# NUS-HPC-AI-Lab/VideoSys

Measured on AMD Instinct MI355X. Metric: videos/min (Open-Sora 512x512x64f, 30 denoise steps, DiT denoising only) + sec/denoise-step, higher is better.
Workload: dtype bf16; 1 GPU; open-sora-v1.2 STDiT3-XL/2 512x512x64f, latent [4,19,64,64], CFG batch 2 = 38912 token rows, 300 text tokens, depth 28; steps_per_video=30, parallelism=dsp1

## Files before the change

### videosys_amd/csrc/rowwise.hip

```cpp
#include "common.h"

#include <cstdlib>
#include "vsys_internal.h"

namespace vsys {
namespace {

template <int MAXV>
__global__ __launch_bounds__(256) void adaln_modulate_kernel(const bf16_t* __restrict__ x, const bf16_t* __restrict__ shift,
                                                             const bf16_t* __restrict__ scale, bf16_t* __restrict__ y,
                                                             int64_t rows, int C, int64_t rows_per_sample,
                                                             int64_t mod_stride, float eps) {
  const int lane = threadIdx.x & 63;
  const int64_t row = (int64_t)blockIdx.x * 4 + (threadIdx.x >> 6);
  if (row >= rows) return;
  const int nchunk = C >> 3;
  const bf16_t* xr = x + row * C;
  float v[MAXV][8];
  float s = 0.f;
#pragma unroll
  for (int i = 0; i < MAXV; ++i) {
    const int c = lane + 64 * i;
    if (c < nchunk) {
      uint4 u = *reinterpret_cast<const uint4*>(xr + c * 8);
      unpack8(u, v[i]);
#pragma unroll
      for (int e = 0; e < 8; ++e) s += v[i][e];
    }
  }
  const float mean = wave_sum(s) / (float)C;
  float q = 0.f;
#pragma unroll
  for (int i = 0; i < MAXV; ++i) {
    const int c = lane + 64 * i;
    if (c < nchunk) {
#pragma unroll
      for (int e = 0; e < 8; ++e) {
        float d = v[i][e] - mean;
        q += d * d;
      }
    }
  }
  const float rstd = rsqrtf(wave_sum(q) / (float)C + eps);
  const int64_t b = row / rows_per_sample;
  const bf16_t* sh = shift + b * mod_stride;
  const bf16_t* sc = scale + b * mod_stride;
  bf16_t* yr = y + row * C;
#pragma unroll
  for (int i = 0; i < MAXV; ++i) {
    const int c = lane + 64 * i;
    if (c < nchunk) {
      float a[8], m[8], o[8];
      unpack8(*reinterpret_cast<const uint4*>(sh + c * 8), a);
      unpack8(*reinterpret_cast<const uint4*>(sc + c * 8), m);
#pragma unroll
      for (int e = 0; e < 8; ++e) o[e] = (v[i][e] - mean) * rstd * (1.0f + m[e]) + a[e];
      *reinterpret_cast<uint4*>(yr + c * 8) = pack8(o);
    }
  }
}

template <int RPW>
__global__ __launch_bounds__(256) void adaln_modulate_rows_kernel(const bf16_t* __restrict__ x, const bf16_t* __restrict__ shift,
                                                                  const bf16_t* __restrict__ scale, bf16_t* __restrict__ y,
                                                                  int64_t rows, int C, int64_t rows_per_sample,
                                                                  int64_t mod_stride, float eps) {
  constexpr int MAXV = 3;
  const int lane = threadIdx.x & 63;
  const int64_t row0 = ((int64_t)blockIdx.x * 4 + (threadIdx.x >> 6)) * RPW;
  if (row0 >= rows) return;
  const int nchunk = C >> 3;
  uint4 u[RPW][MAXV];
#pragma unroll
  for (int r = 0; r < RPW; ++r) {
    const int64_t row = row0 + r < rows ? row0 + r : rows - 1;
#pragma unroll
    for (int i = 0; i < MAXV; ++i) {
      const int c = lane + 64 * i;
      u[r][i] = c < nchunk ? *reinterpret_cast<const uint4*>(x + row * C + c * 8) : make_uint4(0, 0, 0, 0);
    }
  }
  const int64_t b = row0 / rows_per_sample;
  uint4 ush[MAXV], usc[MAXV];
#pragma unroll
  for (int i = 0; i < MAXV; ++i) {
    const int c = lane + 64 * i;
    ush[i] = c < nchunk ? *reinterpret_cast<const uint4*>(shift + b * mod_stride + c * 8) : make_uint4(0, 0, 0, 0);
    usc[i] = c < nchunk ? *reinterpret_cast<const uint4*>(scale + b * mod_stride + c * 8) : make_uint4(0, 0, 0, 0);
  }
#pragma unroll
  for (int r = 0; r < RPW; ++r) {
    float v[MAXV][8];
    float s = 0.f;
#pragma unroll
    for (int i = 0; i < MAXV; ++i) {
      unpack8(u[r][i], v[i]);
      if (lane + 64 * i < nchunk) {
#pragma unroll
        for (int e = 0; e < 8; ++e) s += v[i][e];
      }
    }
    const float mean = wave_sum(s) / (float)C;
    float q = 0.f;
#pragma unroll
    for (int i = 0; i < MAXV; ++i) {
      if (lane + 64 * i < nchunk) {
#pragma unroll
        for (int e = 0; e < 8; ++e) {
          float d = v[i][e] - mean;
          q += d * d;
        }
      }
    }
    const float rstd = rsqrtf(wave_sum(q) / (float)C + eps);
    if (row0 + r < rows) {
#pragma unroll
      for (int i = 0; i < MAXV; ++i) {
        const int c = lane + 64 * i;
        if (c < nchunk) {
          float a[8], m[8], o[8];
          unpack8(ush[i], a);
          unpack8(usc[i], m);
#pragma unroll
          for (int e = 0; e < 8; ++e) o[e] = (v[i][e] - mean) * rstd * (1.0f + m[e]) + a[e];
          *reinterpret_cast<uint4*>(y + (row0 + r) * C + c * 8) = pack8(o);
        }
      }
    }
  }
}

template <int MAXV>
__global__ __launch_bounds__(256) void ln_modulate_kernel(const bf16_t* __restrict__ x, const bf16_t* __restrict__ ln_w,
                                                          const bf16_t* __restrict__ ln_b, const bf16_t* __restrict__ shift,
                                                          const bf16_t* __restrict__ scale, bf16_t* __restrict__ y, int64_t rows,
                                                          int C, int64_t rows_per_sample, int64_t mod_stride, int64_t seg_split,
                                                          int64_t mod_alt, float eps) {
  const int lane = threadIdx.x & 63;
  const int64_t row = (int64_t)blockIdx.x * 4 + (threadIdx.x >> 6);
  if (row >= rows) return;
  const int nchunk = C >> 3;
  const bf16_t* xr = x + row * C;
  float v[MAXV][8];
  float s = 0.f;
#pragma unroll
  for (int i = 0; i < MAXV; ++i) {
    const int c = lane + 64 * i;
    if (c < nchunk) {
      unpack8(*reinterpret_cast<const uint4*>(xr + c * 8), v[i]);
#pragma unroll
      for (int e = 0; e < 8; ++e) s += v[i][e];
    }
  }
  const float mean = wave_sum(s) / (float)C;
  float q = 0.f;
#pragma unroll
  for (int i = 0; i < MAXV; ++i) {
    const int c = lane + 64 * i;
    if (c < nchunk) {
#pragma unroll
      for (int e = 0; e < 8; ++e) {
        const float d = v[i][e] - mean;
        q += d * d;
      }
    }
  }
  const float rstd = rsqrtf(wave_sum(q) / (float)C + eps);
  const int64_t b = row / rows_per_sample;
  const int64_t alt = (seg_split > 0 && row - b * rows_per_sample < seg_split) ? mod_alt : 0;
  bf16_t* yr = y + row * C;
#pragma unroll
  for (int i = 0; i < MAXV; ++i) {
    const int c = lane + 64 * i;
    if (c < nchunk) {
      float o[8];
#pragma unroll
      for (int e = 0; e < 8; ++e) o[e] = (v[i][e] - mean) * rstd;
      if (ln_w != nullptr) {
        float w[8], bb[8];
        unpack8(*reinterpret_cast<const uint4*>(ln_w + c * 8), w);
        unpack8(*reinterpret_cast<const uint4*>(ln_b + c * 8), bb);
#pragma unroll
        for (int e = 0; e < 8; ++e) o[e] = o[e] * w[e] + bb[e];
      }
      if (shift != nullptr) {
        float a[8], m[8];
        unpack8(*reinterpret_cast<const uint4*>(shift + b * mod_stride + alt + c * 8), a);
        unpack8(*reinterpret_cast<const uint4*>(scale + b * mod_stride + alt + c * 8), m);
#pragma unroll
        for (int e = 0; e < 8; ++e) o[e] = o[e] * (1.0f + m[e]) + a[e];
      }
      *reinterpret_cast<uint4*>(yr + c * 8) = pack8(o);
    }
  }
}

__global__ void gate_add_rows_kernel(bf16_t* __restrict__ x, const bf16_t* __restrict__ y, const bf16_t* __restrict__ gate,
                                     int64_t rows, int C8, int64_t rows_per_sample, int64_t gate_stride, int64_t seg_split,
                                     int64_t gate_alt) {
  const int64_t total = rows * C8;
  for (int64_t i = (int64_t)blockIdx.x * blockDim.x + threadIdx.x; i < total; i += (int64_t)gridDim.x * blockDim.x) {
    const int64_t r = i / C8;
    const int c = (int)(i - r * C8);
    const int64_t b = r / rows_per_sample;
    const int64_t alt = (seg_split > 0 && r - b * rows_per_sample < seg_split) ? gate_alt : 0;
    float a[8], v[8], g[8];
    unpack8(reinterpret_cast<const uint4*>(x)[i], a);
    unpack8(reinterpret_cast<const uint4*>(y)[i], v);
    unpack8(*reinterpret_cast<const uint4*>(gate + b * gate_stride + alt + c * 8), g);
#pragma unroll
    for (int k = 0; k < 8; ++k) a[k] += bf2f(f2bf(g[k] * v[k]));
    reinterpret_cast<uint4*>(x)[i] = pack8(a);
  }
}

__global__ void im2col_patch_kernel(const float* __restrict__ z, int Bz, bf16_t* __restrict__ out, int B, int F, int Cin, int H,
                                    int W, int p) {
  const int Hp = H / p, Wp = W / p, K = Cin * p * p;
  const int64_t total = (int64_t)B * F * Hp * Wp * K;
  for (int64_t i = (int64_t)blockIdx.x * blockDim.x + threadIdx.x; i < total; i += (int64_t)gridDim.x * blockDim.x) {
    const int k = (int)(i % K);
    const int64_t tok = i / K;
    const int wp = (int)(tok % Wp), hp = (int)((tok / Wp) % Hp), f = (int)((tok / ((int64_t)Wp * Hp)) % F);
    const int b = (int)(tok / ((int64_t)Wp * Hp * F));
    const int dx = k % p, dy = (k / p) % p, c = k / (p * p);
    out[i] = f2bf(z[((((int64_t)(b % Bz) * F + f) * Cin + c) * H + hp * p + dy) * W + wp * p + dx]);
  }
}

__global__ void unpatchify_cvx_kernel(const bf16_t* __restrict__ x, int64_t ldx, float* __restrict__ out, int B, int F, int Hp,
                                      int Wp, int Cout, int p) {
  const int H = Hp * p, W = Wp * p;
  const int64_t total = (int64_t)B * F * Cout * H * W;
  for (int64_t i = (int64_t)blockIdx.x * blockDim.x + threadIdx.x; i < total; i += (int64_t)gridDim.x * blockDim.x) {
    const int w = (int)(i % W), h = (int)((i / W) % H), c = (int)((i / ((int64_t)W * H)) % Cout);
    const int64_t bf = i / ((int64_t)W * H * Cout);
    const int64_t tok = (bf * Hp + h / p) * Wp + w / p;
    out[i] = bf2f(x[tok * ldx + (c * p + h % p) * p + w % p]);
  }
}

__global__ void mod_table_kernel(const bf16_t* __restrict__ table, const bf16_t* __restrict__ t_mlp, bf16_t* __restrict__ out,
                                 int nblk, int B, int C6) {
  const int64_t i = (int64_t)blockIdx.x * blockDim.x + threadIdx.x;
  const int64_t total = (int64_t)nblk * B * C6;
  if (i >= total) return;
  const int c = (int)(i % C6);
  const int b = (int)((i / C6) % B);
  const int k = (int)(i / ((int64_t)C6 * B));
  out[i] = f2bf(bf2f(table[(int64_t)k * C6 + c]) + bf2f(t_mlp[(int64_t)b * C6 + c]));
}

__global__ void timestep_embedding_kernel(const float* __restrict__ t, bf16_t* __restrict__ out, int B, int dim) {
  const int i = blockIdx.x * blockDim.x + threadIdx.x;
  const int half = dim / 2;
  if (i >= B * half) return;
  const int b = i / half, k = i - b * half;
  const float f = expf(-9.210340371976184f * (float)k / (float)half);
  const float a = t[b] * f;
  out[(int64_t)b * dim + k] = f2bf(cosf(a));
  out[(int64_t)b * dim + half + k] = f2bf(sinf(a));
}

__global__ __launch_bounds__(256) void patch_embed_kernel(const float* __restrict__ x, int Bz, const bf16_t* __restrict__ w,
                                                          const bf16_t* __restrict__ bias, const bf16_t* __restrict__ pos,
                                                          bf16_t* __restrict__ out, int B, int Cin, int T, int H, int W,
                                                          int ph, int pw, int C, int s0, int Sl) {
  const int Hp = (H + ph - 1) / ph, Wp = (W + pw - 1) / pw;
  const int S = Hp * Wp;
  const int cchunks = C >> 3;
  const int64_t total = (int64_t)B * T * Sl * cchunks;
  const int64_t i = (int64_t)blockIdx.x * blockDim.x + threadIdx.x;
  if (i >= total) return;
  const int cc = (int)(i % cchunks);
  const int64_t tok = i / cchunks;
  const int s = s0 + (int)(tok % Sl);
  const int t = (int)((tok / Sl) % T);
  const int b = (int)(tok / ((int64_t)Sl * T));
  const int bz = b % Bz;
  if (s >= S) {
    *reinterpret_cast<uint4*>(out + tok * C + cc * 8) = make_uint4(0, 0, 0, 0);
    return;
  }
  const int hp = s / Wp, wp = s - hp * Wp;
  float acc[8];
  {
    float bb[8];
    unpack8(*reinterpret_cast<const uint4*>(bias + cc * 8), bb);
#pragma unroll
    for (int e = 0; e < 8; ++e) acc[e] = bb[e];
  }
  const int K = Cin * ph * pw;
  if (K == 16) {
    float xin[16];
#pragma unroll
    for (int k = 0; k < 16; ++k) {
      const int ci = k >> 2, dy = (k >> 1) & 1, dx = k & 1;
      const int hh = hp * 2 + dy, ww = wp * 2 + dx;
      xin[k] = 0.f;
      if (ph == 2 && pw == 2 && hh < H && ww < W) xin[k] = bf2f(f2bf(x[((((int64_t)bz * Cin + ci) * T + t) * H + hh) * W + ww]));
    }
    if (ph == 2 && pw == 2) {
#pragma unroll
      for (int e = 0; e < 8; ++e) {
        const bf16_t* wr = w + (int64_t)(cc * 8 + e) * 16;
        float wa[8], wb[8];
        unpack8(*reinterpret_cast<const uint4*>(wr), wa);
        unpack8(*reinterpret_cast<const uint4*>(wr + 8), wb);
#pragma unroll
        for (int k = 0; k < 8; ++k) acc[e] += xin[k] * wa[k] + xin[k + 8] * wb[k];
      }
    }
  }
  if (!(K == 16 && ph == 2 && pw == 2)) {
    for (int ci = 0; ci < Cin; ++ci)
      for (int dy = 0; dy < ph; ++dy)
        for (int dx = 0; dx < pw; ++dx) {
          const int hh = hp * ph + dy, ww = wp * pw + dx;
          float xv = 0.f;
          if (hh < H && ww < W) xv = bf2f(f2bf(x[((((int64_t)bz * Cin + ci) * T + t) * H + hh) * W + ww]));
          const int k = (ci * ph + dy) * pw + dx;
#pragma unroll
          for (int e = 0; e < 8; ++e) acc[e] += xv * bf2f(w[(int64_t)(cc * 8 + e) * K + k]);
        }
  }
  float pp[8];
  unpack8(*reinterpret_cast<const uint4*>(pos + (int64_t)s * C + cc * 8), pp);
#pragma unroll
  for (int e = 0; e < 8; ++e) acc[e] = bf2f(f2bf(acc[e])) + pp[e];
  *reinterpret_cast<uint4*>(out + tok * C + cc * 8) = pack8(acc);
}

template <int MAXV>
__global__ __launch_bounds__(256) void final_layer_kernel(const bf16_t* __restrict__ x, const bf16_t* __restrict__ table,
                                                          const bf16_t* __restrict__ tvec, const bf16_t* __restrict__ w,
                                                          const bf16_t* __restrict__ bias, float* __restrict__ out,
                                                          int B, int T, int Hp, int Wp, int H, int W, int ph, int pw,
                                                          int Cout, int C, float eps, int Sl, float* __restrict__ tokens) {
  const int lane = threadIdx.x & 63;
  const int S = Sl;
  const int64_t rows = (int64_t)B * T * S;
  const int64_t row = (int64_t)blockIdx.x * 4 + (threadIdx.x >> 6);
  if (row >= rows) return;
  const int nchunk = C >> 3;
  const bf16_t* xr = x + row * C;
  float v[MAXV][8];
  float s = 0.f;
#pragma unroll
  for (int i = 0; i < MAXV; ++i) {
    const int c = lane + 64 * i;
    if (c < nchunk) {
      unpack8(*reinterpret_cast<const uint4*>(xr + c * 8), v[i]);
#pragma unroll
      for (int e = 0; e < 8; ++e) s += v[i][e];
    } else {
#pragma unroll
      for (int e = 0; e < 8; ++e) v[i][e] = 0.f;
    }
  }
  const float mean = wave_sum(s) / (float)C;
  float q = 0.f;
#pragma unroll
  for (int i = 0; i < MAXV; ++i) {
    const int c = lane + 64 * i;
    if (c < nchunk) {
#pragma unroll
      for (int e = 0; e < 8; ++e) {
        float d = v[i][e] - mean;
        q += d * d;
      }
    }
  }
  const float rstd = rsqrtf(wave_sum(q) / (float)C + eps);
  const int b = (int)(row / ((int64_t)T * S));
#pragma unroll
  for (int i = 0; i < MAXV; ++i) {
    const int c = lane + 64 * i;
    if (c < nchunk) {
      float sh[8], sc[8], tt[8];
      unpack8(*reinterpret_cast<const uint4*>(table + c * 8), sh);
      unpack8(*reinterpret_cast<const uint4*>(table + C + c * 8), sc);
      unpack8(*reinterpret_cast<const uint4*>(tvec + (int64_t)b * C + c * 8), tt);
#pragma unroll
      for (int e = 0; e < 8; ++e) {
        const float shift = bf2f(f2bf(sh[e] + tt[e])), scale = bf2f(f2bf(sc[e] + tt[e]));
        v[i][e] = bf2f(f2bf((v[i][e] - mean) * rstd * (1.0f + scale) + shift));
      }
    }
  }
  const int NOUT = ph * pw * Cout;
  const int64_t tok = row % ((int64_t)T * S);
  const int t = (int)(tok / S), sidx = (int)(tok % S);
  const int hp = sidx / Wp, wp = sidx - hp * Wp;
  for (int n = 0; n < NOUT; ++n) {
    const bf16_t* wr = w + (int64_t)n * C;
    float d = 0.f;
#pragma unroll
    for (int i = 0; i < MAXV; ++i) {
      const int c = lane + 64 * i;
      if (c < nchunk) {
        float ww[8];
        unpack8(*reinterpret_cast<const uint4*>(wr + c * 8), ww);
#pragma unroll
        for (int e = 0; e < 8; ++e) d += v[i][e] * ww[e];
      }
    }
    d = wave_sum(d);
    if (lane == 0) {
      d = bf2f(f2bf(d + bf2f(bias[n])));
      if (tokens != nullptr) {
        tokens[row * NOUT + n] = d;
        continue;
      }
      const int co = n % Cout;
      const int dx = (n / Cout) % pw, dy = n / (Cout * pw);
      const int hh = hp * ph + dy, ww2 = wp * pw + dx;
      if (hh < H && ww2 < W) out[((((int64_t)b * Cout + co) * T + t) * H + hh) * W + ww2] = d;
    }
  }
}

__global__ void unpatchify_tokens_kernel(const float* __restrict__ tok, float* __restrict__ out, int P, int B, int T, int Sl,
                                         int Hp, int Wp, int H, int W, int ph, int pw, int Cout) {
  const int NOUT = ph * pw * Cout;
  const int64_t total = (int64_t)B * Cout * T * H * W;
  const int64_t i = (int64_t)blockIdx.x * blockDim.x + threadIdx.x;
  if (i >= total) return;
  const int ww = (int)(i % W), hh = (int)((i / W) % H), t = (int)((i / ((int64_t)W * H)) % T);
  const int co = (int)((i / ((int64_t)W * H * T)) % Cout), b = (int)(i / ((int64_t)W * H * T * Cout));
  const int hp = hh / ph, dy = hh - hp * ph, wp = ww / pw, dx = ww - wp * pw;
  const int s = hp * Wp + wp;
  const int r = s / Sl, j = s - r * Sl;
  const int n = (dy * pw + dx) * Cout + co;
  out[i] = tok[((((int64_t)r * B + b) * T + t) * Sl + j) * NOUT + n];
}

__global__ void cfg_euler_kernel(float* __restrict__ z, const float* __restrict__ model_out, int Bz, int Cin, int Cout,
                                 int64_t thw, float guidance, float dt) {
  const int64_t i = (int64_t)blockIdx.x * blockDim.x + threadIdx.x;
  const int64_t total = (int64_t)Bz * Cin * thw;
  if (i >= total) return;
  const int64_t sp = i % thw;
  const int c = (int)((i / thw) % Cin);
  const int b = (int)(i / (thw * Cin));
  const float cond = model_out[((int64_t)b * Cout + c) * thw + sp];
  const float unc = model_out[((int64_t)(b + Bz) * Cout + c) * thw + sp];
  z[i] = z[i] + (unc + guidance * (cond - unc)) * dt;
}

__global__ void cfg_axpby_kernel(float* __restrict__ z, const float* __restrict__ model_out, int Bz, int Cin, int Cout,
                                 int64_t thw, float guidance, float c_z, float c_eps, int cond_first) {
  const int64_t i = (int64_t)blockIdx.x * blockDim.x + threadIdx.x;
  const int64_t total = (int64_t)Bz * Cin * thw;
  if (i >= total) return;
  const int64_t sp = i % thw;
  const int c = (int)((i / thw) % Cin);
  const int b = (int)(i / (thw * Cin));
  const float h0 = model_out[((int64_t)b * Cout + c) * thw + sp];
  const float h1 = model_out[((int64_t)(b + Bz) * Cout + c) * thw + sp];
  const float cond = cond_first ? h0 : h1, unc = cond_first ? h1 : h0;
  z[i] = c_z * z[i] + c_eps * (unc + guidance * (cond - unc));
}

__global__ void add_bcast_rows_kernel(bf16_t* __restrict__ x, const bf16_t* __restrict__ e, int64_t rows, int C8, int64_t group,
                                      int64_t period) {
  const int64_t total = rows * C8;
  for (int64_t i = (int64_t)blockIdx.x * blockDim.x + threadIdx.x; i < total; i += (int64_t)gridDim.x * blockDim.x) {
    const int64_t r = i / C8;
    const int c = (int)(i - r * C8);
    const int64_t er = (r / group) % period;
    float a[8], b[8];
    unpack8(reinterpret_cast<const uint4*>(x)[i], a);
    unpack8(reinterpret_cast<const uint4*>(e)[er * C8 + c], b);
#pragma unroll
    for (int k = 0; k < 8; ++k) a[k] += b[k];
    reinterpret_cast<uint4*>(x)[i] = pack8(a);
  }
}

__global__ void add_rows_kernel(bf16_t* __restrict__ x, const bf16_t* __restrict__ y, int64_t n8) {
  for (int64_t i = (int64_t)blockIdx.x * blockDim.x + threadIdx.x; i < n8; i += (int64_t)gridDim.x * blockDim.x) {
    float a[8], b[8];
    unpack8(reinterpret_cast<const uint4*>(x)[i], a);
    unpack8(reinterpret_cast<const uint4*>(y)[i], b);
#pragma unroll
    for (int e = 0; e < 8; ++e) a[e] += b[e];
    reinterpret_cast<uint4*>(x)[i] = pack8(a);
  }
}

__global__ void scale_add_rows_kernel(const bf16_t* __restrict__ a, int64_t lda, const bf16_t* __restrict__ b, int64_t ldb,
                                      bf16_t* __restrict__ out, int64_t ldo, int64_t rows, int C8, float scale) {
  const int64_t total = rows * C8;
  for (int64_t i = (int64_t)blockIdx.x * blockDim.x + threadIdx.x; i < total; i += (int64_t)gridDim.x * blockDim.x) {
    const int64_t r = i / C8;
    const int c = (int)(i - r * C8) * 8;
    float x[8], y[8];
    unpack8(*reinterpret_cast<const uint4*>(a + r * lda + c), x);
    unpack8(*reinterpret_cast<const uint4*>(b + r * ldb + c), y);
#pragma unroll
    for (int e = 0; e < 8; ++e) x[e] = bf2f(f2bf(x[e] * scale)) + y[e];
    *reinterpret_cast<uint4*>(out + r * ldo + c) = pack8(x);
  }
}

__global__ void copy_4d_kernel(const bf16_t* __restrict__ src, bf16_t* __restrict__ dst, int n0, int n1, int n2, int C,
                               int64_t ss0, int64_t ss1, int64_t ss2, int64_t ds0, int64_t ds1, int64_t ds2,
                               int n1_valid, int n2_valid) {
  const int cch = C >> 3;
  const int64_t total = (int64_t)n0 * n1 * n2 * cch;
  for (int64_t i = (int64_t)blockIdx.x * blockDim.x + threadIdx.x; i < total; i += (int64_t)gridDim.x * blockDim.x) {
    const int c = (int)(i % cch);
    int64_t r = i / cch;
    const int i2 = (int)(r % n2);
    r /= n2;
    const int i1 = (int)(r % n1);
    const int i0 = (int)(r / n1);
    uint4 v = make_uint4(0, 0, 0, 0);
    if (i1 < n1_valid && i2 < n2_valid) v = *reinterpret_cast<const uint4*>(src + i0 * ss0 + i1 * ss1 + i2 * ss2 + c * 8);
    *reinterpret_cast<uint4*>(dst + i0 * ds0 + i1 * ds1 + i2 * ds2 + c * 8) = v;
  }
}

struct CopyBatch {
  int nops;
  CopyDesc d[VSYS_COPY_BATCH_MAX];
};
__global__ void copy_4d_batch_kernel(const bf16_t* __restrict__ src, bf16_t* __restrict__ dst, CopyBatch b) {
  const CopyDesc& o = b.d[blockIdx.y];
  const int cch = o.C >> 3;
  const int64_t total = (int64_t)o.n0 * o.n1 * o.n2 * cch;
  const bf16_t* s = src + o.src_off;
  bf16_t* d = dst + o.dst_off;
  for (int64_t i = (int64_t)blockIdx.x * blockDim.x + threadIdx.x; i < total; i += (int64_t)gridDim.x * blockDim.x) {
    const int c = (int)(i % cch);
    int64_t r = i / cch;
    const int i2 = (int)(r % o.n2);
    r /= o.n2;
    const int i1 = (int)(r % o.n1);
    const int i0 = (int)(r / o.n1);
    uint4 v = make_uint4(0, 0, 0, 0);
    if (i1 < o.n1_valid && i2 < o.n2_valid) v = *reinterpret_cast<const uint4*>(s + i0 * o.ss0 + i1 * o.ss1 + i2 * o.ss2 + c * 8);
    *reinterpret_cast<uint4*>(d + i0 * o.ds0 + i1 * o.ds1 + i2 * o.ds2 + c * 8) = v;
  }
}

}

int launch_copy_4d_batch(const bf16_t* src, bf16_t* dst, const CopyDesc* ops, int nops, hipStream_t stream) {
  if (nops <= 0) return 0;
  if (nops > VSYS_COPY_BATCH_MAX) return VSYS_ERR_SHAPE;
  CopyBatch b;
  b.nops = nops;
  int64_t most = 0;
  for (int i = 0; i < nops; ++i) {
    if (ops[i].C % 8 || ops[i].n0 < 0 || ops[i].n1 < 0 || ops[i].n2 < 0) return VSYS_ERR_SHAPE;
    b.d[i] = ops[i];
    const int64_t t = (int64_t)ops[i].n0 * ops[i].n1 * ops[i].n2 * (ops[i].C / 8);
    most = t > most ? t : most;
  }
  if (most <= 0) return 0;
  int64_t grid = (most + 255) / 256;
  if (grid > 2048) grid = 2048;
  hipLaunchKernelGGL(copy_4d_batch_kernel, dim3((unsigned)grid, (unsigned)nops), dim3(256), 0, stream, src, dst, b);
  return hipGetLastError() == hipSuccess ? 0 : VSYS_ERR_LAUNCH;
}

int launch_adaln_modulate(const bf16_t* x, const bf16_t* shift, const bf16_t* scale, bf16_t* y, int64_t rows, int C,
                          int64_t rows_per_sample, int64_t mod_stride, float eps, hipStream_t stream) {
  if (rows <= 0) return 0;
  if (C % 8 != 0 || C > 64 * 8 * 4 || rows_per_sample <= 0 || (mod_stride % 8)) return VSYS_ERR_SHAPE;
  if (C > 64 * 8 * 2 && C <= 64 * 8 * 3 && rows_per_sample % 2 == 0) {
    hipLaunchKernelGGL(adaln_modulate_rows_kernel<2>, dim3((unsigned)((rows + 7) / 8)), dim3(256), 0, stream, x, shift, scale, y, rows, C,
                       rows_per_sample, mod_stride, eps);
    return hipGetLastError() == hipSuccess ? 0 : VSYS_ERR_LAUNCH;
  }
  const unsigned grid = (unsigned)((rows + 3) / 4);
  if (C <= 64 * 8 * 2)
    hipLaunchKernelGGL(adaln_modulate_kernel<2>, dim3(grid), dim3(256), 0, stream, x, shift, scale, y, rows, C,
                       rows_per_sample, mod_stride, eps);
  else if (C <= 64 * 8 * 3)
    hipLaunchKernelGGL(adaln_modulate_kernel<3>, dim3(grid), dim3(256), 0, stream, x, shift, scale, y, rows, C,
                       rows_per_sample, mod_stride, eps);
  else
    hipLaunchKernelGGL(adaln_modulate_kernel<4>, dim3(grid), dim3(256), 0, stream, x, shift, scale, y, rows, C,
                       rows_per_sample, mod_stride, eps);
  return hipGetLastError() == hipSuccess ? 0 : VSYS_ERR_LAUNCH;
}

int launch_ln_modulate(const bf16_t* x, const bf16_t* ln_w, const bf16_t* ln_b, const bf16_t* shift, const bf16_t* scale,
                       bf16_t* y, int64_t rows, int C, int64_t rows_per_sample, int64_t mod_stride, int64_t seg_split,
                       int64_t mod_alt, float eps, hipStream_t stream) {
  if (rows <= 0) return 0;
  if (C % 8 != 0 || C > 64 * 8 * 6 || rows_per_sample <= 0 || (mod_stride % 8) || (mod_alt % 8)) return VSYS_ERR_SHAPE;
  if ((ln_w == nullptr) != (ln_b == nullptr) || (shift == nullptr) != (scale == nullptr)) return VSYS_ERR_ARG;
  const unsigned grid = (unsigned)((rows + 3) / 4);
#define VSYS_LNMOD(V)                                                                                                      \
  hipLaunchKernelGGL(ln_modulate_kernel<V>, dim3(grid), dim3(256), 0, stream, x, ln_w, ln_b, shift, scale, y, rows, C,       \
                     rows_per_sample, mod_stride, seg_split, mod_alt, eps)
  if (C <= 64 * 8 * 2) VSYS_LNMOD(2);
  else if (C <= 64 * 8 * 3) VSYS_LNMOD(3);
  else if (C <= 64 * 8 * 4) VSYS_LNMOD(4);
  else VSYS_LNMOD(6);
#undef VSYS_LNMOD
  return hipGetLastError() == hipSuccess ? 0 : VSYS_ERR_LAUNCH;
}

int launch_gate_add_rows(bf16_t* x, const bf16_t* y, const bf16_t* gate, int64_t rows, int C, int64_t rows_per_sample,
                         int64_t gate_stride, int64_t seg_split, int64_t gate_alt, hipStream_t stream) {
  if (rows <= 0) return 0;
  if (C % 8 || rows_per_sample <= 0 || (gate_stride % 8) || (gate_alt % 8)) return VSYS_ERR_SHAPE;
  int64_t grid = (rows * (C / 8) + 255) / 256;
  if (grid > 2048 * 4) grid = 2048 * 4;
  hipLaunchKernelGGL(gate_add_rows_kernel, dim3((unsigned)grid), dim3(256), 0, stream, x, y, gate, rows, C / 8, rows_per_sample,
                     gate_stride, seg_split, gate_alt);
  return hipGetLastError() == hipSuccess ? 0 : VSYS_ERR_LAUNCH;
}

int launch_im2col_patch(const float* z, int Bz, bf16_t* out, int B, int F, int Cin, int H, int W, int p, hipStream_t stream) {
  if (p <= 0 || H % p || W % p || Bz <= 0) return VSYS_ERR_SHAPE;
  const int64_t total = (int64_t)B * F * (H / p) * (W / p) * Cin * p * p;
  if (total <= 0) return 0;
  int64_t grid = (total + 255) / 256;
  if (grid > 2048 * 8) grid = 2048 * 8;
  hipLaunchKernelGGL(im2col_patch_kernel, dim3((unsigned)grid), dim3(256), 0, stream, z, Bz, out, B, F, Cin, H, W, p);
  return hipGetLastError() == hipSuccess ? 0 : VSYS_ERR_LAUNCH;
}

int launch_unpatchify_cvx(const bf16_t* x, int64_t ldx, float* out, int B, int F, int Hp, int Wp, int Cout, int p,
                          hipStream_t stream) {
  const int64_t total = (int64_t)B * F * Cout * Hp * p * Wp * p;
  if (total <= 0) return 0;
  int64_t grid = (total + 255) / 256;
  if (grid > 2048 * 8) grid = 2048 * 8;
  hipLaunchKernelGGL(unpatchify_cvx_kernel, dim3((unsigned)grid), dim3(256), 0, stream, x, ldx, out, B, F, Hp, Wp, Cout, p);
  return hipGetLastError() == hipSuccess ? 0 : VSYS_ERR_LAUNCH;
}

int launch_mod_table(const bf16_t* table, const bf16_t* t_mlp, bf16_t* out, int nblk, int B, int C6, hipStream_t stream) {
  const int64_t total = (int64_t)nblk * B * C6;
  if (total <= 0) return 0;
  hipLaunchKernelGGL(mod_table_kernel, dim3((unsigned)((total + 255) / 256)), dim3(256), 0, stream, table, t_mlp, out, nblk,
                     B, C6);
  return hipGetLastError() == hipSuccess ? 0 : VSYS_ERR_LAUNCH;
}

int launch_timestep_embedding(const float* t, bf16_t* out, int B, int dim, hipStream_t stream) {
  if (dim % 2) return VSYS_ERR_SHAPE;
  const int total = B * (dim / 2);
  if (total <= 0) return 0;
  hipLaunchKernelGGL(timestep_embedding_kernel, dim3((total + 127) / 128), dim3(128), 0, stream, t, out, B, dim);
  return hipGetLastError() == hipSuccess ? 0 : VSYS_ERR_LAUNCH;
}

int launch_patch_embed(const float* x, int Bz, const bf16_t* w, const bf16_t* bias, const bf16_t* pos, bf16_t* out, int B,
                       int Cin, int T, int H, int W, int ph, int pw, int C, int s0, int Sl, hipStream_t stream) {
  if (C % 8 || Bz <= 0 || s0 < 0) return VSYS_ERR_SHAPE;
  const int Hp = (H + ph - 1) / ph, Wp = (W + pw - 1) / pw;
  if (Sl < 0) Sl = Hp * Wp;
  const int64_t total = (int64_t)B * T * Sl * (C / 8);
  if (total <= 0) return 0;
  if ((total + 255) / 256 > 0x7fffffff) return VSYS_ERR_SHAPE;
  hipLaunchKernelGGL(patch_embed_kernel, dim3((unsigned)((total + 255) / 256)), dim3(256), 0, stream, x, Bz, w, bias, pos, out,
                     B, Cin, T, H, W, ph, pw, C, s0, Sl);
  return hipGetLastError() == hipSuccess ? 0 : VSYS_ERR_LAUNCH;
}

int launch_unpatchify_tokens(const float* tok, float* out, int P, int B, int T, int Sl, int Hp, int Wp, int H, int W, int ph,
                             int pw, int Cout, hipStream_t stream) {
  if (P <= 0 || Sl <= 0 || (int64_t)P * Sl < (int64_t)Hp * Wp) return VSYS_ERR_SHAPE;
  const int64_t total = (int64_t)B * Cout * T * H * W;
  if (total <= 0) return 0;
  if ((total + 255) / 256 > 0x7fffffff) return VSYS_ERR_SHAPE;
  hipLaunchKernelGGL(unpatchify_tokens_kernel, dim3((unsigned)((total + 255) / 256)), dim3(256), 0, stream, tok, out, P, B, T, Sl,
                     Hp, Wp, H, W, ph, pw, Cout);
  return hipGetLastError() == hipSuccess ? 0 : VSYS_ERR_LAUNCH;
}

int launch_final_layer(const bf16_t* x, const bf16_t* table, const bf16_t* tvec, const bf16_t* w, const bf16_t* bias,
                       float* out, int B, int T, int Hp, int Wp, int H, int W, int ph, int pw, int Cout, int C, float eps,
                       int Sl, float* tokens, hipStream_t stream) {
  if (C % 8 != 0 || C > 64 * 8 * 4) return VSYS_ERR_SHAPE;
  if (Sl < 0) Sl = Hp * Wp;
  if (tokens == nullptr && Sl != Hp * Wp) return VSYS_ERR_ARG;
  const int64_t rows = (int64_t)B * T * Sl;
  if (rows <= 0) return 0;
  const unsigned grid = (unsigned)((rows + 3) / 4);
  if (C <= 64 * 8 * 2)
    hipLaunchKernelGGL(final_layer_kernel<2>, dim3(grid), dim3(256), 0, stream, x, table, tvec, w, bias, out, B, T, Hp, Wp,
                       H, W, ph, pw, Cout, C, eps, Sl, tokens);
  else if (C <= 64 * 8 * 3)
    hipLaunchKernelGGL(final_layer_kernel<3>, dim3(grid), dim3(256), 0, stream, x, table, tvec, w, bias, out, B, T, Hp, Wp,
                       H, W, ph, pw, Cout, C, eps, Sl, tokens);
  else
    hipLaunchKernelGGL(final_layer_kernel<4>, dim3(grid), dim3(256), 0, stream, x, table, tvec, w, bias, out, B, T, Hp, Wp,
                       H, W, ph, pw, Cout, C, eps, Sl, tokens);
  return hipGetLastError() == hipSuccess ? 0 : VSYS_ERR_LAUNCH;
}

int launch_cfg_euler(float* z, const float* model_out, int Bz, int Cin, int Cout, int64_t thw, float guidance, float dt,
                     hipStream_t stream) {
  const int64_t total = (int64_t)Bz * Cin * thw;
  if (total <= 0) return 0;
  hipLaunchKernelGGL(cfg_euler_kernel, dim3((unsigned)((total + 255) / 256)), dim3(256), 0, stream, z, model_out, Bz, Cin,
                     Cout, thw, guidance, dt);
  return hipGetLastError() == hipSuccess ? 0 : VSYS_ERR_LAUNCH;
}

int launch_cfg_axpby(float* z, const float* model_out, int Bz, int Cin, int Cout, int64_t thw, float guidance, float c_z,
                     float c_eps, int cond_first, hipStream_t stream) {
  const int64_t total = (int64_t)Bz * Cin * thw;
  if (total <= 0) return 0;
  hipLaunchKernelGGL(cfg_axpby_kernel, dim3((unsigned)((total + 255) / 256)), dim3(256), 0, stream, z, model_out, Bz, Cin,
                     Cout, thw, guidance, c_z, c_eps, cond_first);
  return hipGetLastError() == hipSuccess ? 0 : VSYS_ERR_LAUNCH;
}

int launch_add_bcast_rows(bf16_t* x, const bf16_t* e, int64_t rows, int C, int64_t group, int64_t period, hipStream_t stream) {
  if (rows <= 0) return 0;
  if (C % 8 || group <= 0 || period <= 0) return VSYS_ERR_SHAPE;
  int64_t grid = (rows * (C / 8) + 255) / 256;
  if (grid > 2048 * 4) grid = 2048 * 4;
  hipLaunchKernelGGL(add_bcast_rows_kernel, dim3((unsigned)grid), dim3(256), 0, stream, x, e, rows, C / 8, group, period);
  return hipGetLastError() == hipSuccess ? 0 : VSYS_ERR_LAUNCH;
}

int launch_add_rows(bf16_t* x, const bf16_t* y, int64_t n, hipStream_t stream) {
  if (n <= 0) return 0;
  if (n % 8) return VSYS_ERR_SHAPE;
  const int64_t n8 = n / 8;
  int64_t grid = (n8 + 255) / 256;
  if (grid > 2048 * 4) grid = 2048 * 4;
  hipLaunchKernelGGL(add_rows_kernel, dim3((unsigned)grid), dim3(256), 0, stream, x, y, n8);
  return hipGetLastError() == hipSuccess ? 0 : VSYS_ERR_LAUNCH;
}

int launch_scale_add_rows(const bf16_t* a, int64_t lda, const bf16_t* b, int64_t ldb, bf16_t* out, int64_t ldo, int64_t rows, int C,
                          float scale, hipStream_t stream) {
  if (rows < 0 || C < 0) return VSYS_ERR_SHAPE;
  if (rows == 0 || C == 0) return 0;
  if (C % 8 || lda < C || ldb < C || ldo < C) return VSYS_ERR_SHAPE;
  if ((lda % 8) || (ldb % 8) || (ldo % 8) || reinterpret_cast<uintptr_t>(a) % 16 || reinterpret_cast<uintptr_t>(b) % 16 ||
      reinterpret_cast<uintptr_t>(out) % 16)
    return VSYS_ERR_ALIGN;
  int64_t grid = (rows * (C / 8) + 255) / 256;
  if (grid > 2048 * 4) grid = 2048 * 4;
  hipLaunchKernelGGL(scale_add_rows_kernel, dim3((unsigned)grid), dim3(256), 0, stream, a, lda, b, ldb, out, ldo, rows, C / 8, scale);
  return hipGetLastError() == hipSuccess ? 0 : VSYS_ERR_LAUNCH;
}

int launch_copy_4d(const bf16_t* src, bf16_t* dst, int n0, int n1, int n2, int C, int64_t ss0, int64_t ss1, int64_t ss2,
                   int64_t ds0, int64_t ds1, int64_t ds2, int n1_valid, int n2_valid, hipStream_t stream) {
  if (C % 8) return VSYS_ERR_SHAPE;
  const int64_t total = (int64_t)n0 * n1 * n2 * (C / 8);
  if (total <= 0) return 0;
  int64_t grid = (total + 255) / 256;
  if (grid > 2048 * 4) grid = 2048 * 4;
  hipLaunchKernelGGL(copy_4d_kernel, dim3((unsigned)grid), dim3(256), 0, stream, src, dst, n0, n1, n2, C, ss0, ss1, ss2, ds0,
                     ds1, ds2, n1_valid, n2_valid);
  return hipGetLastError() == hipSuccess ? 0 : VSYS_ERR_LAUNCH;
}

}
```

Before: 20.77 videos/min.

## Add specialized patch-embed and final-layer kernels with LDS weight reuse

Adds a patch-embed kernel specialized for Cin=4, 2x2 patches. It stages input patches in shared memory and keeps the projection weights in registers across many tokens, instead of re-reading weights per output element. It also adds a final-layer kernel that caches the 32-row output weights and per-sample modulation in LDS. That kernel processes two rows per wave with prefetch and uses a reduce-scatter shuffle so lanes finish the 32 dot products together. Both kernels run only at the start and end of each denoise step, so any gain is bounded by their small share of DiT time; an env flag restores the old paths.

```diff
diff --git a/videosys_amd/csrc/rowwise.hip b/videosys_amd/csrc/rowwise.hip
--- a/videosys_amd/csrc/rowwise.hip
+++ b/videosys_amd/csrc/rowwise.hip
@@ -331,6 +331,104 @@
   *reinterpret_cast<uint4*>(out + tok * C + cc * 8) = pack8(acc);
 }
 
+constexpr int PE_NT = 128;
+constexpr int PE_TL = 16;
+__global__ __launch_bounds__(256, 2) void patch_embed_run_kernel(const float* __restrict__ x, int Bz, const bf16_t* __restrict__ w,
+                                                                 const bf16_t* __restrict__ bias, const bf16_t* __restrict__ pos,
+                                                                 bf16_t* __restrict__ out, int T, int H, int W, int C, int s0,
+                                                                 int Sl, int64_t ntok, int wgs_per_chunk) {
+#pragma clang fp contract(off)
+  constexpr int Cin = 4;
+  __shared__ __attribute__((aligned(16))) float xs[PE_NT * 16];
+  __shared__ int64_t xoff_s[PE_NT];
+  __shared__ int s_s[PE_NT], hp_s[PE_NT], wp_s[PE_NT];
+  const int tid = threadIdx.x;
+  const int Hp = (H + 1) / 2, Wp = (W + 1) / 2;
+  const int S = Hp * Wp;
+  const int chunk = blockIdx.x / wgs_per_chunk, part = blockIdx.x - chunk * wgs_per_chunk;
+  const int64_t t0 = (int64_t)chunk * PE_NT;
+  if (tid < PE_NT) {
+    const int64_t tok = t0 + tid;
+    int s = -2, hp = 0, wp = 0;
+    int64_t xoff = 0;
+    if (tok < ntok) {
+      s = s0 + (int)(tok % Sl);
+      if (s < S) {
+        const int t = (int)((tok / Sl) % T);
+        const int b = (int)(tok / ((int64_t)Sl * T));
+        const int bz = b % Bz;
+        hp = s / Wp;
+        wp = s - hp * Wp;
+        xoff = ((((int64_t)bz * Cin) * T + t) * H + hp * 2) * W + wp * 2;
+      } else {
+        s = -1;
+      }
+    }
+    s_s[tid] = s;
+    hp_s[tid] = hp;
+    wp_s[tid] = wp;
+    xoff_s[tid] = xoff;
+  }
+  __syncthreads();
+  {
+    const int j = tid >> 1, dx = tid & 1;
+    const int s = s_s[j];
+    const int ww = wp_s[j] * 2 + dx;
+    const int hh0 = hp_s[j] * 2;
+    const int64_t xoff = xoff_s[j];
+    const int64_t plane = (int64_t)T * H * W;
+#pragma unroll
+    for (int p = 0; p < 8; ++p) {
+      const int ci = p >> 1, dy = p & 1;
+      const bool ok = s >= 0 && hh0 + dy < H && ww < W;
+      const float xv = bf2f(f2bf(x[xoff + ci * plane + (ok ? dy * W + dx : 0)]));
+      xs[j * 16 + ci * 4 + dy * 2 + dx] = ok ? xv : 0.f;
+    }
+  }
+  __syncthreads();
+  const int cchunks = C >> 3;
+  const int f = part * 256 + tid;
+  if (f >= PE_TL * cchunks) return;
+  const int tl = f / cchunks, cc = f - tl * cchunks;
+  float bb[8], wa[8][8], wb[8][8];
+  unpack8(*reinterpret_cast<const uint4*>(bias + cc * 8), bb);
+#pragma unroll
+  for (int e = 0; e < 8; ++e) {
+    const bf16_t* wr = w + (int64_t)(cc * 8 + e) * 16;
+    unpack8(*reinterpret_cast<const uint4*>(wr), wa[e]);
+    unpack8(*reinterpret_cast<const uint4*>(wr + 8), wb[e]);
+  }
+  for (int j = tl; j < PE_NT; j += PE_TL) {
+    const int s = s_s[j];
+    if (s == -2) break;
+    bf16_t* orow = out + (t0 + j) * C + cc * 8;
+    if (s < 0) {
+      *reinterpret_cast<uint4*>(orow) = make_uint4(0, 0, 0, 0);
+      continue;
+    }
+    const uint4 pu = *reinterpret_cast<const uint4*>(pos + (int64_t)s * C + cc * 8);
+    float xin[16];
+#pragma unroll
+    for (int k4 = 0; k4 < 4; ++k4) {
+      const float4 v4 = *reinterpret_cast<const float4*>(xs + j * 16 + k4 * 4);
+      xin[k4 * 4 + 0] = v4.x; xin[k4 * 4 + 1] = v4.y; xin[k4 * 4 + 2] = v4.z; xin[k4 * 4 + 3] = v4.w;
+    }
+    float acc[8];
+#pragma unroll
+    for (int e = 0; e < 8; ++e) acc[e] = bb[e];
+#pragma unroll
+    for (int e = 0; e < 8; ++e) {
+#pragma unroll
+      for (int k = 0; k < 8; ++k) acc[e] += __builtin_fmaf(xin[k], wa[e][k], xin[k + 8] * wb[e][k]);
+    }
+    float pp[8];
+    unpack8(pu, pp);
+#pragma unroll
+    for (int e = 0; e < 8; ++e) acc[e] = bf2f(f2bf(acc[e])) + pp[e];
+    *reinterpret_cast<uint4*>(orow) = pack8(acc);
+  }
+}
+
 template <int MAXV>
 __global__ __launch_bounds__(256) void final_layer_kernel(const bf16_t* __restrict__ x, const bf16_t* __restrict__ table,
                                                           const bf16_t* __restrict__ tvec, const bf16_t* __restrict__ w,
@@ -416,6 +514,183 @@
       const int dx = (n / Cout) % pw, dy = n / (Cout * pw);
       const int hh = hp * ph + dy, ww2 = wp * pw + dx;
       if (hh < H && ww2 < W) out[((((int64_t)b * Cout + co) * T + t) * H + hh) * W + ww2] = d;
+    }
+  }
+}
+
+template <int HALF>
+__device__ __forceinline__ void reduce_scatter_step(float* d, int lane) {
+  const bool up = (lane & (2 * HALF)) != 0;
+#pragma unroll
+  for (int n = 0; n < HALF; ++n) {
+    const float send = up ? d[n] : d[n + HALF];
+    const float keep = up ? d[n + HALF] : d[n];
+    d[n] = keep + __shfl_xor(send, 2 * HALF, 64);
+  }
+}
+__device__ __forceinline__ void wave_sum32_scatter(float* d, int lane) {
+  reduce_scatter_step<16>(d, lane);
+  reduce_scatter_step<8>(d, lane);
+  reduce_scatter_step<4>(d, lane);
+  reduce_scatter_step<2>(d, lane);
+  reduce_scatter_step<1>(d, lane);
+  d[0] += __shfl_xor(d[0], 1, 64);
+}
+
+template <int MAXV, int RPW>
+__global__ __launch_bounds__(256, 2) void final_layer_rows_kernel(const bf16_t* __restrict__ x, const bf16_t* __restrict__ table,
+                                                                  const bf16_t* __restrict__ tvec, const bf16_t* __restrict__ w,
+                                                                  const bf16_t* __restrict__ bias, float* __restrict__ out, int T,
+                                                                  int Wp, int H, int W, int ph, int pw, int Cout, int C, float eps,
+                                                                  int Sl, float* __restrict__ tokens, int rows_per_wg,
+                                                                  int wgs_per_sample) {
+#pragma clang fp contract(off)
+  static_assert(RPW == 1 || RPW == 2, "a lane pair holds each total: one row per lane parity at most");
+  constexpr int NOUT = 32;
+  extern __shared__ __attribute__((aligned(16))) char smem[];
+  bf16_t* ws = reinterpret_cast<bf16_t*>(smem);
+  bf16_t* mods = ws + NOUT * C;
+  float* bs = reinterpret_cast<float*>(mods + 2 * C);
+  const int tid = threadIdx.x, lane = tid & 63, wave = tid >> 6;
+  const int nchunk = C >> 3;
+  const int b = blockIdx.x / wgs_per_sample, part = blockIdx.x - b * wgs_per_sample;
+  const int S = Sl;
+  const int TS = T * S;
+  const int lr0 = part * rows_per_wg;
+  const int lr1 = lr0 + rows_per_wg < TS ? lr0 + rows_per_wg : TS;
+  for (int i = tid; i < NOUT * nchunk; i += 256) reinterpret_cast<uint4*>(ws)[i] = reinterpret_cast<const uint4*>(w)[i];
+  for (int c = tid; c < nchunk; c += 256) {
+    float sh[8], sc[8], tt[8], shift[8], scale[8];
+    unpack8(*reinterpret_cast<const uint4*>(table + c * 8), sh);
+    unpack8(*reinterpret_cast<const uint4*>(table + C + c * 8), sc);
+    unpack8(*reinterpret_cast<const uint4*>(tvec + (int64_t)b * C + c * 8), tt);
+#pragma unroll
+    for (int e = 0; e < 8; ++e) {
+      shift[e] = sh[e] + tt[e];
+      scale[e] = sc[e] + tt[e];
+    }
+    reinterpret_cast<uint4*>(mods)[c] = pack8(shift);
+    reinterpret_cast<uint4*>(mods + C)[c] = pack8(scale);
+  }
+  if (tid < NOUT) bs[tid] = bf2f(bias[tid]);
+  __syncthreads();
+
+  const bf16_t* xb = x + (int64_t)b * TS * C;
+  int cl[MAXV];
+#pragma unroll
+  for (int i = 0; i < MAXV; ++i) cl[i] = lane + 64 * i < nchunk ? lane + 64 * i : nchunk - 1;
+  uint4 u[RPW][MAXV];
+#pragma unroll
+  for (int r = 0; r < RPW; ++r) {
+    int lr = lr0 + wave * RPW + r;
+    lr = lr < lr1 ? lr : lr1 - 1;
+#pragma unroll
+    for (int i = 0; i < MAXV; ++i) u[r][i] = *reinterpret_cast<const uint4*>(xb + (int64_t)lr * C + cl[i] * 8);
+  }
+  for (int g0 = lr0 + wave * RPW; g0 < lr1; g0 += 4 * RPW) {
+    uint4 un[RPW][MAXV];
+#pragma unroll
+    for (int r = 0; r < RPW; ++r) {
+      int lr = g0 + 4 * RPW + r;
+      lr = lr < lr1 ? lr : lr1 - 1;
+#pragma unroll
+      for (int i = 0; i < MAXV; ++i) un[r][i] = *reinterpret_cast<const uint4*>(xb + (int64_t)lr * C + cl[i] * 8);
+    }
+    float v[RPW][MAXV][8];
+    float mean[RPW], rstd[RPW];
+#pragma unroll
+    for (int r = 0; r < RPW; ++r) {
+      float s = 0.f;
+#pragma unroll
+      for (int i = 0; i < MAXV; ++i) {
+        const int c = lane + 64 * i;
+        if (c < nchunk) {
+          unpack8(u[r][i], v[r][i]);
+#pragma unroll
+          for (int e = 0; e < 8; ++e) s += v[r][i][e];
+        } else {
+#pragma unroll
+          for (int e = 0; e < 8; ++e) v[r][i][e] = 0.f;
+        }
+      }
+      mean[r] = wave_sum(s) / (float)C;
+      float q = 0.f;
+#pragma unroll
+      for (int i = 0; i < MAXV; ++i) {
+        const int c = lane + 64 * i;
+        if (c < nchunk) {
+#pragma unroll
+          for (int e = 0; e < 8; ++e) {
+            float d = v[r][i][e] - mean[r];
+            q += d * d;
+          }
+        }
+      }
+      rstd[r] = rsqrtf(wave_sum(q) / (float)C + eps);
+    }
+#pragma unroll
+    for (int i = 0; i < MAXV; ++i) {
+      const int c = lane + 64 * i;
+      if (c < nchunk) {
+        float shift[8], scale[8];
+        unpack8(reinterpret_cast<const uint4*>(mods)[c], shift);
+        unpack8(reinterpret_cast<const uint4*>(mods + C)[c], scale);
+#pragma unroll
+        for (int r = 0; r < RPW; ++r) {
+#pragma unroll
+          for (int e = 0; e < 8; ++e)
+            v[r][i][e] = bf2f(f2bf(__builtin_fmaf((v[r][i][e] - mean[r]) * rstd[r], 1.0f + scale[e], shift[e])));
+        }
+      }
+    }
+    float d[RPW][NOUT];
+    uint4 wq[MAXV];
+#pragma unroll
+    for (int i = 0; i < MAXV; ++i) wq[i] = *reinterpret_cast<const uint4*>(ws + cl[i] * 8);
+#pragma unroll
+    for (int n = 0; n < NOUT; ++n) {
+      uint4 wnx[MAXV];
+#pragma unroll
+      for (int i = 0; i < MAXV; ++i) wnx[i] = *reinterpret_cast<const uint4*>(ws + (n + 1 < NOUT ? n + 1 : n) * C + cl[i] * 8);
+#pragma unroll
+      for (int r = 0; r < RPW; ++r) d[r][n] = 0.f;
+#pragma unroll
+      for (int i = 0; i < MAXV; ++i) {
+        float ww[8];
+        unpack8(wq[i], ww);
+#pragma unroll
+        for (int r = 0; r < RPW; ++r) {
+#pragma unroll
+          for (int e = 0; e < 8; ++e) d[r][n] = __builtin_fmaf(v[r][i][e], ww[e], d[r][n]);
+        }
+      }
+#pragma unroll
+      for (int i = 0; i < MAXV; ++i) wq[i] = wnx[i];
+      __builtin_amdgcn_sched_barrier(0);
+    }
+#pragma unroll
+    for (int r = 0; r < RPW; ++r) wave_sum32_scatter(d[r], lane);
+    const int n = lane >> 1;
+    const int mine = RPW == 2 ? (lane & 1) : 0;
+    const int lr = g0 + mine;
+    if (lr < lr1 && (RPW == 2 || (lane & 1) == 0)) {
+      float y = RPW == 2 && mine ? d[RPW - 1][0] : d[0][0];
+      y = bf2f(f2bf(y + bs[n]));
+      if (tokens != nullptr) {
+        tokens[((int64_t)b * TS + lr) * NOUT + n] = y;
+      } else {
+        const int t = lr / S, sidx = lr - t * S;
+        const int hp = sidx / Wp, wp = sidx - hp * Wp;
+        const int co = n % Cout;
+        const int dx = (n / Cout) % pw, dy = n / (Cout * pw);
+        const int hh = hp * ph + dy, ww2 = wp * pw + dx;
+        if (hh < H && ww2 < W) out[((((int64_t)b * Cout + co) * T + t) * H + hh) * W + ww2] = y;
+      }
+    }
+#pragma unroll
+    for (int r = 0; r < RPW; ++r) {
+#pragma unroll
+      for (int i = 0; i < MAXV; ++i) u[r][i] = un[r][i];
     }
   }
 }
@@ -545,6 +820,33 @@
   }
 }
 
+bool rowwise_v1() {
+  static const bool on = [] { const char* e = getenv("VSYS_ROWWISE_V1"); return e && e[0] == '1'; }();
+  return on;
+}
+
+template <int MAXV, int RPW>
+int launch_final_layer_rows(const bf16_t* x, const bf16_t* table, const bf16_t* tvec, const bf16_t* w, const bf16_t* bias, float* out,
+                            int B, int T, int Wp, int H, int W, int ph, int pw, int Cout, int C, float eps, int Sl, float* tokens,
+                            hipStream_t stream) {
+  const int lds = 68 * C + 128;
+  static const bool attr_ok = [] {
+    return hipFuncSetAttribute((const void*)final_layer_rows_kernel<MAXV, RPW>, hipFuncAttributeMaxDynamicSharedMemorySize,
+                               68 * 64 * 8 * MAXV + 128) == hipSuccess;
+  }();
+  if (!attr_ok) return VSYS_ERR_LAUNCH;
+  const int TS = T * Sl;
+  int per = B > 0 ? 512 / B : 1;
+  per = per > 0 ? per : 1;
+  int rows_per_wg = (TS + per - 1) / per;
+  rows_per_wg = rows_per_wg > 32 ? rows_per_wg : 32;
+  rows_per_wg = (rows_per_wg + 4 * RPW - 1) / (4 * RPW) * (4 * RPW);
+  const int wgs_per_sample = (TS + rows_per_wg - 1) / rows_per_wg;
+  hipLaunchKernelGGL((final_layer_rows_kernel<MAXV, RPW>), dim3((unsigned)(B * wgs_per_sample)), dim3(256), lds, stream, x, table,
+                     tvec, w, bias, out, T, Wp, H, W, ph, pw, Cout, C, eps, Sl, tokens, rows_per_wg, wgs_per_sample);
+  return hipGetLastError() == hipSuccess ? 0 : VSYS_ERR_LAUNCH;
+}
+
 }
 
 int launch_copy_4d_batch(const bf16_t* src, bf16_t* dst, const CopyDesc* ops, int nops, hipStream_t stream) {
@@ -661,6 +963,16 @@
   const int64_t total = (int64_t)B * T * Sl * (C / 8);
   if (total <= 0) return 0;
   if ((total + 255) / 256 > 0x7fffffff) return VSYS_ERR_SHAPE;
+  if (!rowwise_v1() && Cin == 4 && ph == 2 && pw == 2 && T > 0 && H > 0 && W > 0) {
+    const int64_t ntok = (int64_t)B * T * Sl;
+    const int wgs_per_chunk = (PE_TL * (C / 8) + 255) / 256;
+    const int64_t grid = (ntok + PE_NT - 1) / PE_NT * wgs_per_chunk;
+    if (grid <= 0x7fffffff) {
+      hipLaunchKernelGGL(patch_embed_run_kernel, dim3((unsigned)grid), dim3(256), 0, stream, x, Bz, w, bias, pos, out, T, H, W, C,
+                         s0, Sl, ntok, wgs_per_chunk);
+      return hipGetLastError() == hipSuccess ? 0 : VSYS_ERR_LAUNCH;
+    }
+  }
   hipLaunchKernelGGL(patch_embed_kernel, dim3((unsigned)((total + 255) / 256)), dim3(256), 0, stream, x, Bz, w, bias, pos, out,
                      B, Cin, T, H, W, ph, pw, C, s0, Sl);
   return hipGetLastError() == hipSuccess ? 0 : VSYS_ERR_LAUNCH;
@@ -685,6 +997,13 @@
   if (tokens == nullptr && Sl != Hp * Wp) return VSYS_ERR_ARG;
   const int64_t rows = (int64_t)B * T * Sl;
   if (rows <= 0) return 0;
+  if (!rowwise_v1() && ph * pw * Cout == 32 && (int64_t)T * Sl <= 0x7fffffff) {
+    if (C <= 64 * 8 * 2)
+      return launch_final_layer_rows<2, 2>(x, table, tvec, w, bias, out, B, T, Wp, H, W, ph, pw, Cout, C, eps, Sl, tokens, stream);
+    if (C <= 64 * 8 * 3)
+      return launch_final_layer_rows<3, 2>(x, table, tvec, w, bias, out, B, T, Wp, H, W, ph, pw, Cout, C, eps, Sl, tokens, stream);
+    return launch_final_layer_rows<4, 1>(x, table, tvec, w, bias, out, B, T, Wp, H, W, ph, pw, Cout, C, eps, Sl, tokens, stream);
+  }
   const unsigned grid = (unsigned)((rows + 3) / 4);
   if (C <= 64 * 8 * 2)
     hipLaunchKernelGGL(final_layer_kernel<2>, dim3(grid), dim3(256), 0, stream, x, table, tvec, w, bias, out, B, T, Hp, Wp,
```

New measurement: 20.91 videos/min, median of 6. About the same (+0.7%).
